# bing164/PL-VI-ORBSLAM3

Hardware: AMD Instinct MI355X
Metric: frames/sec ORB+LSD extract+match, 640×480 mono, 1/2/4/8 MI355X (higher is better)
Workload: dtype u8; 1 GPU; C1+C2+C3: ORB extract (1000 feats, 1.2, 8 levels, FAST 20/7) || LSD+LBD (200 lines, scale 0.8, 2 octaves) as one HIP-stream schedule, then ORB kNN-2 + LineMatcher::match vs previous frame; batch=3072, width=640, height=480, parallelism=sequence-sharded x1, gather=False, inflight=2

## Files before the change

include/plvi_frontend.h:

```cpp
#ifndef PLVI_FRONTEND_H
#define PLVI_FRONTEND_H

#include <stddef.h>
#include <stdint.h>

#ifdef __cplusplus
extern "C" {
#endif

enum {
  PLVI_OK = 0,
  PLVI_E_EMPTY = -1,
  PLVI_E_BADARG = -2,
  PLVI_E_CAPACITY = -3,
  PLVI_E_HIP = -4,
  PLVI_E_OVERFLOW = -5,
  PLVI_E_SIZE = -6,
  PLVI_E_CAPTURE = -7,
};

enum {
  PLVI_COMPAT_GAUSS_ROUNDED = 1,
  PLVI_COMPAT_RESIZE_V_GENERIC = 2,
  PLVI_COMPAT_EXP_CV_TABLE = 4,
// ... 52 lines not shown
                     int* cap);

int plvi_orb_pyramid_level(plvi_orb_extractor* h, int frame, int level, uint8_t* dst, int* w, int* hgt);

int plvi_orb_pyramid_device(plvi_orb_extractor* h, int level, const uint8_t** d_frame0, size_t* frame_stride, int* w,
                            int* hgt, int* nlevels);

int plvi_orb_scale_tables(plvi_orb_extractor* h, float* scale, float* inv_scale, float* sigma2, float* inv_sigma2);

int plvi_orb_level_quota(plvi_orb_extractor* h, int* quota);

int plvi_orb_profile(plvi_orb_extractor* h, int enable);
int plvi_orb_profile_read(plvi_orb_extractor* h, float* stage_ms, int* runs);

int plvi_orb_kernel_timing(plvi_orb_extractor* h, int enable);
int plvi_orb_kernel_timing_read(plvi_orb_extractor* h, float* total_ms, int* launches);
int plvi_orb_kernel_timing_read_kind(plvi_orb_extractor* h, int kind, float* total_ms, int* launches);
int plvi_orb_debug_node_cap(plvi_orb_extractor* h, int cap);

typedef struct plvi_line_extractor plvi_line_extractor;

typedef struct plvi_line_params {
  int nfeatures;
  int refine;
  float lsd_scale;
  int nlevels;
  float scale;
  int extractor;
  unsigned compat;
} plvi_line_params;

int plvi_lines_create(const plvi_line_params* p, int width, int height, int max_batch, int device,
                      plvi_line_extractor** out);
int plvi_lines_destroy(plvi_line_extractor* h);

int plvi_lines_extract(plvi_line_extractor* h, const uint8_t* img, int width, int height, size_t stride,
                       plvi_keyline* keylines, uint8_t* desc, double* line_fns, int cap, int* n);

int plvi_lines_extract_batch(plvi_line_extractor* h, const uint8_t* d_frames, int n_frames, size_t frame_stride,
                             size_t row_stride, void* stream);
int plvi_lines_outputs(plvi_line_extractor* h, plvi_keyline** d_kl, uint8_t** d_desc, double** d_fn, int** d_count,
                       int* cap);
int plvi_lines_errors(plvi_line_extractor* h, int* frame_flags, int* any, void* stream);

int plvi_lines_pyramid_level(plvi_line_extractor* h, int frame, int level, uint8_t* dst, int* w, int* hgt);

int plvi_lines_scale_tables(plvi_line_extractor* h, float* scale, float* inv_scale, float* sigma2, float* inv_sigma2);

int plvi_lines_profile(plvi_line_extractor* h, int enable);
int plvi_lines_debug_stats(plvi_line_extractor* h, unsigned long long* d_stats);
int plvi_lines_debug_mw_stats(plvi_line_extractor* h, int* d_stats);
int plvi_lines_debug_planes(plvi_line_extractor* h, int frame, int octave, float* deg, double* modgrad, float* cs,
                            int* sw, int* sh);
int plvi_lines_debug_sobel(plvi_line_extractor* h, int frame, int octave, short* dxdy, int* w, int* hgt);
int plvi_lines_debug_raw_lines(plvi_line_extractor* h, int frame, int octave, float* out, int cap, int* n);
int plvi_lines_profile_read(plvi_line_extractor* h, float* stage_ms, int* runs);
int plvi_lines_kernel_timing(plvi_line_extractor* h, int enable);
int plvi_lines_kernel_timing_read(plvi_line_extractor* h, float* total_ms, int* launches);
int plvi_lines_kernel_timing_read_kind(plvi_line_extractor* h, int kind, float* total_ms, int* launches);


int plvi_hamming_knn2_batch(const uint8_t* d_q, const int* d_nq, int nq_cap, const uint8_t* d_t, const int* d_nt,
                            int nt_cap, int n_pairs, int* d_idx0, int* d_d0, int* d_idx1, int* d_d1, void* stream);

int plvi_hamming_knn2(const uint8_t* q, int nq, const uint8_t* t, int nt, int* idx0, int* d0, int* idx1, int* d1);

int plvi_line_match_nnr(const uint8_t* desc1, int n1, const uint8_t* desc2, int n2, float nnr, int* matches_12);

int plvi_line_match(const uint8_t* desc1, int n1, const uint8_t* desc2, int n2, float nnr, int* matches_12);

int plvi_line_match_nnr_inout(const uint8_t* desc1, int n1, const uint8_t* desc2, int n2, float nnr, int* matches_12,
                              int n_prev);
int plvi_line_match_inout(const uint8_t* desc1, int n1, const uint8_t* desc2, int n2, float nnr, int* matches_12,
                          int n_prev);

int plvi_line_match_batch(const uint8_t* d_desc1, const int* d_n1, int cap1, const uint8_t* d_desc2, const int* d_n2,
                          int cap2, int n_pairs, float nnr, int* d_scratch, int* d_matches_12, int* d_nmatch,
                          void* stream);

int plvi_descriptor_distance_batch(const uint8_t* d_a, const uint8_t* d_b, int n, int line_matcher_quirk, int* d_out,
                                   void* stream);

int plvi_search_by_bow(float nnratio, int check_orientation, const uint8_t* kf_desc, const float* kf_angle,
                       const uint8_t* kf_live, int kf_n, const int* kf_node, const int* kf_off, int kf_nnodes,
                       const int* kf_idx, const uint8_t* f_desc, const float* f_angle, int f_n, const int* f_node,
                       const int* f_off, int f_nnodes, const int* f_idx, int* match_kf);

int plvi_search_by_bow_batch(int n_pairs, float nnratio, int check_orientation, int kf_cap, int f_cap, int node_cap,
                             const uint8_t* d_kf_desc, const float* d_kf_angle, const uint8_t* d_kf_live,
                             const int* d_kf_node, const int* d_kf_off, const int* d_kf_nnodes, const int* d_kf_idx,
                             const uint8_t* d_f_desc, const float* d_f_angle, const int* d_f_n, const int* d_f_node,
                             const int* d_f_off, const int* d_f_nnodes, const int* d_f_idx, int* d_match_kf,
                             int* d_nmatches, void* stream);

int plvi_search_by_bow_stereo(float nnratio, int check_orientation, const uint8_t* kf_desc, const float* kf_angle,
                              const uint8_t* kf_live, int kf_n, const int* kf_node, const int* kf_off, int kf_nnodes,
                              const int* kf_idx, const uint8_t* f_desc, const float* f_angle, int f_n,
                              const int* f_node, const int* f_off, int f_nnodes, const int* f_idx, int f_nleft,
                              int* match_kf);
int plvi_search_by_bow_stereo_batch(int n_pairs, float nnratio, int check_orientation, int kf_cap, int f_cap,
                                    int node_cap, const uint8_t* d_kf_desc, const float* d_kf_angle,
                                    const uint8_t* d_kf_live, const int* d_kf_node, const int* d_kf_off,
                                    const int* d_kf_nnodes, const int* d_kf_idx, const uint8_t* d_f_desc,
                                    const float* d_f_angle, const int* d_f_n, const int* d_f_node, const int* d_f_off,
                                    const int* d_f_nnodes, const int* d_f_idx, const int* d_f_nleft, int* d_match_kf,
                                    int* d_nmatches, void* stream);
// ... 547 lines not shown
```

pl-vi-orbslam3_amd/csrc/lines_device.h:

```cpp
#pragma once
#include <cstdint>

namespace plvi {

constexpr int kLineMaxOct = 2;
constexpr int kLsdRawCap = 8192;
constexpr int kPrepBands = 8;
constexpr int kPrepBandMax = 256;


struct LineOctDev {
    int w, h;
    long long off;
    long long plane;
    int sw, sh;
    long long soff;
    long long splane;
    int min_reg_size;
    float octaveScale;
    int maxWH;
    long long tabXofs, tabXa, tabYrow, tabYb;
    int xmax;
    long long tabStrips;
    int nstrips;
    long long tabBands1, tabBandsK;
    int lw, lh;
    long long loff, lplane;
};

struct LsdLine {
    float x1, y1, x2, y2;
};

struct LsdRegion {
    int start, n;
    double angle;
};

struct LsdPix {
    float deg;
    float c, s;
    float pad;
};

}
```

pl-vi-orbslam3_amd/csrc/lines_kernels.hpp:

```cpp
#include <hip/hip_runtime.h>

#include "lines_device.h"
#include "plvi_common.h"
#include "plvi_math.h"
#include "std_sort.h"

namespace plvi {

constexpr double kNotdef = -1024.0;
constexpr float kNotdefF = -1024.0f;
constexpr double kD2R = 3.14159265358979323846 / 180;
constexpr double kPi = 3.14159265358979323846;
constexpr double kLog10Of11 = 0x1.0a98b6050c56fp+0;

__global__ __launch_bounds__(256) void lsd_half_kernel(const uint8_t* __restrict__ src, size_t s_frame, size_t s_row,
                                                       uint8_t* __restrict__ dst, int dw, int dh, size_t d_frame) {
    const int f = blockIdx.y;
    const int i = blockIdx.x * 256 + threadIdx.x;
    if (i >= dw * dh) return;
    const int y = i / dw, x = i % dw;
    const uint8_t* S0 = src + (size_t)f * s_frame + (size_t)(2 * y) * s_row;
    const uint8_t* S1 = S0 + s_row;
    const int s = S0[2 * x] + S0[2 * x + 1] + S1[2 * x] + S1[2 * x + 1];
    const int simd = (dw / 8) * 8;
    int v = x < simd ? (s + 2) >> 2 : (int)__builtin_rintf((float)s * 0.25f);
    dst[(size_t)f * d_frame + (size_t)y * dw + x] = (uint8_t)min(max(v, 0), 255);
}

__device__ __forceinline__ int readlane_i(int v, int l) { return __builtin_amdgcn_readlane(v, l); }
__device__ __forceinline__ float readlane_f(float v, int l) {
    return __int_as_float(__builtin_amdgcn_readlane(__float_as_int(v), l));
}
__device__ __forceinline__ double readlane_d(double v, int l) {
    const long long b = __double_as_longlong(v);
    const int lo = __builtin_amdgcn_readlane((int)(b & 0xffffffff), l);
    const int hi = __builtin_amdgcn_readlane((int)(b >> 32), l);
    return __longlong_as_double(((long long)hi << 32) | (unsigned)lo);
}
__device__ __forceinline__ double shfl_d(double v, int src) {
    const long long b = __double_as_longlong(v);
    const int lo = __shfl((int)(b & 0xffffffff), src);
    const int hi = __shfl((int)(b >> 32), src);
    return __longlong_as_double(((long long)hi << 32) | (unsigned)lo);
}

__device__ __forceinline__ int dpp_from_right(int v) {
    return __builtin_amdgcn_update_dpp(0, v, 0x130, 0xf, 0xf, false);
}
__device__ __forceinline__ int dpp_from_left(int v) {
    return __builtin_amdgcn_update_dpp(0, v, 0x138, 0xf, 0xf, false);
}
__device__ __forceinline__ double dpp_from_right_d(double v) {
    const long long b = __double_as_longlong(v);
    const int lo = dpp_from_right((int)(b & 0xffffffff)), hi = dpp_from_right((int)(b >> 32));
    return __longlong_as_double(((long long)hi << 32) | (unsigned)lo);
}

__global__ __launch_bounds__(64) void lsd_prep_kernel(const uint8_t* __restrict__ src, size_t s_frame, size_t s_row,
                                                       int gw, int gh, int sw, int sh, const int4* __restrict__ strips,
                                                       const int4* __restrict__ bands,
                                                       const int* __restrict__ xofs, const float* __restrict__ xa,
                                                       int xmax, const int* __restrict__ yrow,
                                                       const float* __restrict__ yb, double k0, double k1, double k2,
                                                       double k3, double rho, float* __restrict__ pix,
                                                       double* __restrict__ modgrad, float2* __restrict__ pixcs,
                                                       size_t p_frame) {
    __shared__ int hostdx[64];
    const int4 sd = strips[blockIdx.x];
    const int f = blockIdx.y;
    const int4 bd = bands[blockIdx.z];
    const int dyA = bd.x, dyB = bd.y, ybase0 = bd.z;
    const int dyEnd = dyB < sh ? dyB + 1 : sh;
    const int X0 = sd.x, X1 = sd.y, gx0 = sd.z, nc = sd.w;
    const int lane = threadIdx.x;
    const int Lt = xofs[X0 + min(lane, nc - 1)] - gx0 + 3;
    hostdx[lane] = -1;
    __builtin_amdgcn_wave_barrier();
    __builtin_amdgcn_fence(__ATOMIC_ACQ_REL, "wavefront");
    if (lane < nc) hostdx[Lt] = X0 + lane;
    __builtin_amdgcn_wave_barrier();
    __builtin_amdgcn_fence(__ATOMIC_ACQ_REL, "wavefront");
    const int hdx = hostdx[lane];
    const bool interp = hdx >= 0 && hdx < xmax;
    const double a0 = interp ? (double)xa[2 * hdx] : 1.0, a1 = interp ? (double)xa[2 * hdx + 1] : 0.0;
    const uint8_t* S = src + (size_t)f * s_frame + reflect101(gx0 - 3 + lane, gw);
    const int nout = X1 - X0;
    float* P = pix + (size_t)f * p_frame + X0;
    double* M = modgrad + (size_t)f * p_frame + X0;
    float2* CS = pixcs + (size_t)f * p_frame + X0;
    const int yend = gh + 3;
    uint32_t pb[7];
#pragma unroll
    for (int k = 0; k < 7; ++k) pb[k] = S[(size_t)reflect101(ybase0 + k, gh) * s_row];
    double Hw[7];
    double Gprev = 0.0, Gprevn = 0.0, Sp = 0.0, Spn = 0.0;
    int dy = dyA;
    auto emit = [&](int y, double Sc, double Scn) {
        if (lane >= nout) return;
        const int x = X0 + lane;
        float deg = kNotdefF;
        double norm = 0.0;
        if (x < sw - 1 && y < sh - 1) {
            const double DA = Scn - Sp;
            const double BC = Spn - Sc;
            const double gx = DA + BC, gy = DA - BC;
            norm = __builtin_sqrt(rfma(gx, gx, gy * gy) / 4);
            if (!(norm <= rho)) deg = plvi_fast_atan2((float)gx, (float)-gy);
        }
        const size_t o = (size_t)y * sw + lane;
        P[o] = deg;
        M[o] = norm;
        if (deg != kNotdefF) {
            float ps, pc;
            plvi_sincosf_pos((float)((double)deg * kD2R), &ps, &pc);
            CS[o] = make_float2(pc, ps);
        }
    };
    for (int ybase = ybase0; ybase < yend && dy < dyEnd; ybase += 7) {
#pragma unroll
        for (int k = 0; k < 7; ++k) {
            const int y = ybase + k;
            if (y >= yend || dy >= dyEnd) break;
            const int v0 = (int)pb[k];
            if (y + 7 < yend) pb[k] = S[(size_t)reflect101(y + 7, gh) * s_row];
            const int r1 = dpp_from_right(v0), r2 = dpp_from_right(r1), r3 = dpp_from_right(r2);
            const int l1 = dpp_from_left(v0), l2 = dpp_from_left(l1), l3 = dpp_from_left(l2);
            double s = k0 * (double)l3;
            s += k1 * (double)l2;
            s += k2 * (double)l1;
            s += k3 * (double)v0;
            s += k2 * (double)r1;
            s += k1 * (double)r2;
            s += k0 * (double)r3;
            Hw[k] = s;
            const int g = y - 3;
            if (g < ybase0 + 3) continue;
            double G = k3 * Hw[(k + 4) % 7] + 0.0;
            G += k2 * (Hw[(k + 5) % 7] + Hw[(k + 3) % 7]);
            G += k1 * (Hw[(k + 6) % 7] + Hw[(k + 2) % 7]);
            G += k0 * (Hw[k] + Hw[(k + 1) % 7]);
            const double Gn = dpp_from_right_d(G);
            while (dy < dyEnd && yrow[2 * dy + 1] == g) {
                const bool same = yrow[2 * dy] == g;
                const double G0 = same ? G : Gprev, G0n = same ? Gn : Gprevn;
                const double b0 = (double)yb[2 * dy], b1 = (double)yb[2 * dy + 1];
                double H0, H1;
                if (interp) {
                    H0 = G0 * a0 + G0n * a1;
                    H1 = G * a0 + Gn * a1;
                } else {
                    H0 = G0 * 1.0;
                    H1 = G * 1.0;
                }
                const double Sv = H0 * b0 + H1 * b1;
                const double Sc = shfl_d(Sv, Lt);
                const double Scn = dpp_from_right_d(Sc);
                if (dy > dyA) emit(dy - 1, Sc, Scn);
                Sp = Sc;
                Spn = Scn;
                ++dy;
            }
            Gprev = G;
            Gprevn = Gn;
        }
    }
    if (dyB == sh) emit(sh - 1, 0.0, 0.0);
}


struct GrowCtx {
    const float* P;
    unsigned* gbits;
    lds_u32* bits;
    lds_u32* qlds;
    unsigned* qglob;
    lds_f32* win;
    int sw, sh, R, RB, wpr, wb, wbb, QL, ys;
};

typedef unsigned short plvi_u16x2 __attribute__((ext_vector_type(2)));
__device__ __forceinline__ unsigned long long dup_lanes(unsigned pv, int nb, int bp, int nx, int ny) {
    const unsigned pn1 = (unsigned)(nx + 1) | ((unsigned)(ny + 1) << 16);
    const int s = 3 * ny + nx + 4;
    unsigned long long dup = 0;
    for (int p2 = 0; p2 < nb - 1; ++p2) {
        const unsigned q2 = (unsigned)__builtin_amdgcn_readlane((int)pv, 9 * p2);
        const int t2 = 3 * (int)(q2 >> 16) + (int)(q2 & 0xffffu);
        const plvi_u16x2 d = __builtin_bit_cast(plvi_u16x2, pn1) - __builtin_bit_cast(plvi_u16x2, q2);
        const plvi_u16x2 m = __builtin_elementwise_max(d, (plvi_u16x2){2, 2});
        const bool hit = (p2 < bp) & (__builtin_bit_cast(unsigned, m) == 0x00020002u);
        const unsigned long long hm = 0ull - (unsigned long long)hit;
        dup |= (1ull << ((9 * p2 - t2 + s) & 63)) & hm;
    }
    return dup;
}

__device__ __forceinline__ unsigned long long ballot(bool b) { return __builtin_amdgcn_ballot_w64(b); }
__device__ __forceinline__ int mbcnt64(unsigned long long m) {
    return (int)__builtin_amdgcn_mbcnt_hi((unsigned)(m >> 32), __builtin_amdgcn_mbcnt_lo((unsigned)m, 0u));
}
__device__ __forceinline__ unsigned gload_l2(unsigned* p) {
    return __hip_atomic_load(p, __ATOMIC_RELAXED, __HIP_MEMORY_SCOPE_AGENT);
}
__device__ __forceinline__ void gstore_l2(unsigned* p, unsigned v) {
    __hip_atomic_store(p, v, __ATOMIC_RELAXED, __HIP_MEMORY_SCOPE_AGENT);
}
__device__ __forceinline__ void vm_drain() { __builtin_amdgcn_s_waitcnt(0); }

__device__ __forceinline__ bool used_get(const GrowCtx& g, int x, int y) {
    const bool inwin = y < g.wbb + g.RB;
    const int yy = inwin ? y : g.wbb;
    unsigned v = g.bits[(yy & (g.RB - 1)) * g.wpr + (x >> 5)];
    if (__builtin_expect(!inwin, 0)) v = gload_l2(g.gbits + (size_t)y * g.wpr + (x >> 5));
    return y < g.ys || ((v >> (x & 31)) & 1u);
}
__device__ __forceinline__ void used_set(const GrowCtx& g, int x, int y) {
    const unsigned b = 1u << (x & 31);
    if (__builtin_expect(y < g.wbb + g.RB, 1))
// ... 1133 lines not shown
```

pl-vi-orbslam3_amd/csrc/lines_pipeline.hip:

```cpp
#include <hip/hip_runtime.h>

#include <algorithm>
#include <cmath>
#include <cstdlib>
#include <cstring>
#include <memory>
#include <vector>

#include "lines_device.h"
#include "lines_kernels.hpp"
#include "lsd_grow_mw.hpp"
#include "plvi_common.h"

extern "C" int plvi_orb_internal_blur_event(plvi_orb_extractor* h, hipEvent_t ev);
extern "C" int plvi_orb_internal_stage_event(plvi_orb_extractor* h, int stage, hipEvent_t ev);

namespace plvi {

static inline int lround_h(float v) { return (int)lrintf(v); }
static inline int lround_h(double v) { return (int)lrint(v); }
static inline int lfloor_h(float v) { int i = (int)v; return i - (i > v); }

static double cv_exp64f(double x) {
    const double a0s = .9670371139572337719125840413672004409288e-2;
    const double k5 = .99999999999999999998285227504999 / a0s, k4 = .69314718055994546743029643825322 / a0s,
                 k3 = .24022650695886477918181338054308 / a0s, k2 = .55504108793649567998466049042729e-1 / a0s,
                 k1 = .96180973140732918010002372686186e-2 / a0s, k0 = .13369713757180123244806654839424e-2 / a0s;
    const double pre = 1.4426950408889634073599246810019 * 64;
    double y = x * pre;
    const int v = (int)lrint(y);
    int e = (v >> 6) + 1023;
    e = e < 0 ? 0 : e > 2047 ? 2047 : e;
    const double p2 = std::ldexp(1.0, e - 1023);
    const double tab = (double)exp2l((long double)(v & 63) / 64.0L) * a0s;
    y = (y - v) * (1. / 64);
    return p2 * tab * (((((k0 * y + k1) * y + k2) * y + k3) * y + k4) * y + k5);
}

static void gauss_kernel_f64(int n, double sigma, double* k, bool cvExp) {
    const double scale2X = -0.125 / (sigma * sigma);
    const int n2 = (n - 1) / 2;
    std::vector<double> values(n2 + 1);
    double sum = 0;
    for (int i = 0, x = 1 - n; i < n2; ++i, x += 2) {
        const double a = (double)(x * x) * scale2X;
        double t = cvExp ? cv_exp64f(a) : std::exp(a);
        values[i] = t;
        sum += t;
    }
    sum *= 2;
    sum += 1.0;
    const double mul1 = 1.0 / sum;
    for (int i = 0; i < n2; ++i) k[i] = k[n - 1 - i] = values[i] * mul1;
    k[n2] = 1.0 * mul1;
}

struct LinePipeline {
    plvi_line_params prm{};
    int W = 0, H = 0, Bcap = 0, device = 0, nOct = 0, fcap = 0;
    hipStream_t stream = nullptr;
    hipStream_t aux[2] = {nullptr, nullptr};
    hipEvent_t evSobelGo = nullptr;
    hipEvent_t evFork = nullptr, evPrep = nullptr, evSobel = nullptr, evOrb = nullptr, evCrit = nullptr,
               evBlur = nullptr, evGate = nullptr, evGrow2 = nullptr, evPair = nullptr;
    bool growAfterBlur = true, sobelWithGrow = false, growSplit = false;
    int sobelGate = -1;
    bool sobelAfterGrow = false;
    hipStream_t critStream = nullptr;
    hipStream_t crit2 = nullptr;
    hipStream_t octStream = nullptr;
    int orbAfterPrep = 1;
    std::vector<LineOctDev> oct;
    std::vector<float> scaleF, invScaleF;
    double SCALE = 0.8, prec = 0, rho = 0, min_length = 0;
    double gk[7]{};
    int lbdTaps[3] = {14, 62, 104};
    DevBuf d_oct, d_tabs, octImg, pix, modg, seedcs, gbits, qspill, regs, regpts, rawLines, nlines, klTmp, klOut, fnOut, cntOut, descOut, lbdBlur,
        lbdG, err, staging, mwOwn, mwSlot, mwGrow, sortPos;
    size_t qspillFrame = 0, gbitsFrame = 0, lbdPlaneTotal = 0;
    int lastFrames = 0;
    static constexpr int kStages = 5, kRing = 512;
    bool prof = false;
    int profRuns = 0;
    std::vector<hipEvent_t> evs;

    static constexpr int kKRing = 4096;
    bool ktime = false;
    int kn = 0;
    std::vector<hipEvent_t> kev;
    std::vector<hipEvent_t> kevS[3];
    int knS[3] = {0, 0, 0};
    int ktiming(int on) {
        if (on && kev.empty()) {
            kev.resize(2 * kKRing);
            for (auto& e : kev) PLVI_CHECK(hipEventCreate(&e));
            for (auto& v : kevS) {
                v.resize(2 * kKRing);
                for (auto& e : v) PLVI_CHECK(hipEventCreate(&e));
            }
        }
        ktime = on != 0;
        if (on) kn = knS[0] = knS[1] = knS[2] = 0;
        return PLVI_OK;
    }
    void ktimeS(int k, int edge, hipStream_t st) {
        if (!ktime || knS[k] >= kKRing) return;
        (void)hipEventRecord(kevS[k][2 * knS[k] + edge], st);
// ... 81 lines not shown
        SCALE = (double)p->lsd_scale;
        if (!(SCALE > 0) || SCALE > 1) return PLVI_E_BADARG;
        const double ANG_TH = 22.5, QUANT = 2.0, SIGMA_SCALE = 0.6;
        prec = M_PI * ANG_TH / 180;
        const double pp = ANG_TH / 180;
        rho = QUANT / std::sin(prec);
        min_length = 0.025 * std::min(W, H);
        const double sigma = (SCALE < 1) ? (SIGMA_SCALE / SCALE) : SIGMA_SCALE;
        const unsigned hk = (unsigned)std::ceil(sigma * std::sqrt(2 * 3.0 * std::log(10.0)));
        if (SCALE != 1 && 1 + 2 * hk != 7) return PLVI_E_BADARG;
        gauss_kernel_f64(7, sigma, gk, (p->compat & PLVI_COMPAT_EXP_CV_TABLE) != 0);
        if (SCALE == 1) gk[0] = gk[1] = gk[2] = 0.0, gk[3] = 1.0;
        lbdTaps[0] = 14;
        lbdTaps[1] = (p->compat & PLVI_COMPAT_GAUSS_ROUNDED) ? 63 : 62;
        lbdTaps[2] = (p->compat & PLVI_COMPAT_GAUSS_ROUNDED) ? 103 : 104;
        scaleF.assign(nOct, 1.f); invScaleF.assign(nOct, 1.f);
        for (int l = 0; l < nOct; ++l) {
            if (l > 0) scaleF[l] = scaleF[l - 1] * p->scale;
            invScaleF[l] = 1.0f / scaleF[l];
        }
        oct.resize(nOct);
        size_t imgOff = 0, sOff = 0, lOff = 0, maxSplane = 0;
        std::vector<uint8_t> tabs;
        auto put = [&](const void* src, size_t n) {
            size_t o = (tabs.size() + 15) & ~size_t(15);
            tabs.resize(o + n);
            std::memcpy(tabs.data() + o, src, n);
            return (long long)o;
        };
        for (int l = 0; l < nOct; ++l) {
            LineOctDev& d = oct[l];
            std::memset(&d, 0, sizeof(d));
            d.w = lround_h((float)W * invScaleF[l]);
            d.h = lround_h((float)H * invScaleF[l]);
            if (l > 0) {
                if (d.w * 2 != oct[l - 1].w || d.h * 2 != oct[l - 1].h) return PLVI_E_BADARG;
                if (std::fabs(scaleF[l] / scaleF[l - 1] - 2.0f) > 0) return PLVI_E_BADARG;
            }
            d.plane = (long long)d.w * d.h;
            d.off = (long long)imgOff;
            if (l > 0) imgOff += (size_t)d.plane * Bcap;
            d.sw = SCALE != 1 ? lround_h(d.w * SCALE) : d.w;
            d.sh = SCALE != 1 ? lround_h(d.h * SCALE) : d.h;
            d.splane = (long long)d.sw * d.sh;
            d.soff = (long long)sOff;
            sOff += (size_t)d.splane * Bcap;
            maxSplane = std::max(maxSplane, (size_t)d.splane);
            const double LOG_NT = rfma(5 * (std::log10((double)d.sw) + std::log10((double)d.sh)), 0.5,
                                       kLog10Of11);
            d.min_reg_size = (int)(-LOG_NT / std::log10(pp));
            d.octaveScale = (float)std::pow(p->scale, l);
            d.maxWH = std::max(d.w, d.h);
            {
                const double sx = 1. / SCALE, sy = 1. / SCALE;
                std::vector<int> xofs(d.sw), yrow(2 * d.sh);
                std::vector<float> xa(2 * d.sw), yb(2 * d.sh);
                int xmax = d.sw;
                for (int dx = 0; dx < d.sw; ++dx) {
                    float fx = (float)((dx + 0.5) * sx - 0.5);
                    int s = lfloor_h(fx);
                    fx -= s;
                    if (s < 0) { fx = 0; s = 0; }
                    if (s + 1 >= d.w) {
                        xmax = std::min(xmax, dx);
                        if (s >= d.w - 1) { fx = 0; s = d.w - 1; }
                    }
                    xofs[dx] = s;
                    xa[2 * dx] = 1.f - fx;
                    xa[2 * dx + 1] = fx;
                }
                for (int dy = 0; dy < d.sh; ++dy) {
                    float fy = (float)((dy + 0.5) * sy - 0.5);
                    int s = lfloor_h(fy);
                    fy -= s;
                    yrow[2 * dy] = std::min(std::max(s, 0), d.h - 1);
                    yrow[2 * dy + 1] = std::min(std::max(s + 1, 0), d.h - 1);
                    yb[2 * dy] = 1.f - fy;
                    yb[2 * dy + 1] = fy;
                }
                d.xmax = xmax;
                std::vector<int> strips;
                for (int X0 = 0; X0 < d.sw;) {
                    const int gx0 = xofs[X0];
                    int E = X0;
                    while (E < d.sw && xofs[E] + (E < xmax ? 1 : 0) - gx0 + 3 <= 60) ++E;
                    const int X1 = E == d.sw ? E : E - 1;
                    if (X1 <= X0) return PLVI_E_BADARG;
                    strips.insert(strips.end(), {X0, X1, gx0, E - X0});
                    X0 = X1;
                }
                for (int dy = 0; dy < d.sh; ++dy) {
                    const int r1 = yrow[2 * dy + 1], r0 = yrow[2 * dy];
                    if (r0 > r1 || r1 - r0 > 1 || (dy > 0 && r1 < yrow[2 * dy - 1])) return PLVI_E_BADARG;
                }
                d.nstrips = (int)strips.size() / 4;
                d.tabStrips = put(strips.data(), strips.size() * 4);
                for (int nb : {1, kPrepBands}) {
                    std::vector<int> bands;
                    for (int b = 0; b < nb; ++b) {
                        const int dyA = (int)((long long)d.sh * b / nb), dyB = (int)((long long)d.sh * (b + 1) / nb);
                        bands.insert(bands.end(), {dyA, dyB, dyA == 0 ? -3 : yrow[2 * dyA] - 3, 0});
                    }
                    (nb == 1 ? d.tabBands1 : d.tabBandsK) = put(bands.data(), bands.size() * 4);
                }
                d.tabXofs = put(xofs.data(), xofs.size() * 4);
                d.tabXa = put(xa.data(), xa.size() * 4);
                d.tabYrow = put(yrow.data(), yrow.size() * 4);
                d.tabYb = put(yb.data(), yb.size() * 4);
            }
            d.lw = l == 0 ? W : oct[l - 1].lw / 2;
            d.lh = l == 0 ? H : oct[l - 1].lh / 2;
            d.lplane = (long long)d.lw * d.lh;
            d.loff = (long long)lOff;
            lOff += (size_t)d.lplane * Bcap;
        }
        lbdPlaneTotal = lOff;
        qspillFrame = (maxSplane + 1) & ~size_t(1);
        for (auto& d : oct) gbitsFrame = std::max(gbitsFrame, (size_t)d.sh * (size_t)((d.sw + 31) / 32));
        if (d_oct.alloc(sizeof(LineOctDev) * nOct) || d_tabs.alloc(tabs.size())) return PLVI_E_HIP;
        PLVI_CHECK(hipMemcpy(d_oct.p, oct.data(), sizeof(LineOctDev) * nOct, hipMemcpyHostToDevice));
        PLVI_CHECK(hipMemcpy(d_tabs.p, tabs.data(), tabs.size(), hipMemcpyHostToDevice));
        {
            float gL[21], gG[63];
            double u = (7 * 3 - 1) / 2, sg = (7 * 2 + 1) / 2, inv = -1 / (2 * sg * sg);
            for (int i = 0; i < 21; ++i) { double dis = i - u; gL[i] = (float)std::exp(dis * dis * inv); }
            u = (9 * 7 - 1) / 2; sg = u; inv = -1 / (2 * sg * sg);
            for (int i = 0; i < 63; ++i) { double dis = i - u; gG[i] = (float)std::exp(dis * dis * inv); }
            static const unsigned char comb[64] = {0, 1, 0, 2, 0, 3, 0, 4, 0, 5, 0, 6, 1, 2, 1, 3, 1, 4, 1, 5, 1, 6,
                                                   2, 3, 2, 4, 2, 5, 2, 6, 2, 7, 2, 8, 3, 4, 3, 5, 3, 6, 3, 7, 3, 8,
                                                   4, 5, 4, 6, 4, 7, 4, 8, 5, 6, 5, 7, 5, 8, 6, 7, 6, 8, 7, 8};
            PLVI_CHECK(hipMemcpyToSymbol(HIP_SYMBOL(c_gaussL), gL, sizeof(gL)));
            PLVI_CHECK(hipMemcpyToSymbol(HIP_SYMBOL(c_gaussG), gG, sizeof(gG)));
            PLVI_CHECK(hipMemcpyToSymbol(HIP_SYMBOL(c_comb), comb, sizeof(comb)));
        }
        if (octImg.alloc(std::max<size_t>(imgOff, 16)) || pix.alloc(sizeof(float) * sOff) ||
            modg.alloc(sizeof(double) * sOff) || seedcs.alloc(sizeof(float2) * sOff) ||
            gbits.alloc(sizeof(unsigned) * gbitsFrame * nOct * Bcap) || qspill.alloc(sizeof(unsigned) * qspillFrame * nOct * Bcap) ||
            rawLines.alloc(sizeof(LsdLine) * (size_t)kLsdRawCap * nOct * Bcap) ||
            regs.alloc(sizeof(LsdRegion) * (size_t)kLsdRawCap * nOct * Bcap) ||
            regpts.alloc(sizeof(unsigned) * qspillFrame * nOct * Bcap) ||
            nlines.alloc(sizeof(int) * nOct * Bcap) || klTmp.alloc(sizeof(plvi_keyline) * (size_t)kKlCap * Bcap) ||
            sortPos.alloc(sizeof(unsigned short) * 2 * (size_t)kKlCap * Bcap) ||
            klOut.alloc(sizeof(plvi_keyline) * (size_t)fcap * Bcap) || fnOut.alloc(sizeof(double) * 3 * fcap * Bcap) ||
            cntOut.alloc(sizeof(int) * Bcap) || descOut.alloc((size_t)32 * fcap * Bcap) ||
            lbdBlur.alloc((size_t)W * H * Bcap) || lbdG.alloc(sizeof(short2) * lbdPlaneTotal) ||
            err.alloc(sizeof(int) * Bcap) || staging.alloc((size_t)W * H))
            return PLVI_E_HIP;
        PLVI_CHECK(hipMemset(err.p, 0, sizeof(int) * Bcap));
        size_t maxSw = 0;
        for (auto& d : oct) maxSw = std::max(maxSw, (size_t)d.sw);
        const size_t wprMax = (maxSw + 31) / 32;
        size_t budget = 6 * 1024;
        if (const char* e = getenv("PLVI_GROW_LDS")) budget = (size_t)atol(e);
        budget = std::min<size_t>(budget, 160 * 1024);
        growRB = 64;
        if (const char* e = getenv("PLVI_GROW_RB")) growRB = atoi(e);
        if (growRB < 2 || (growRB & (growRB - 1)) || growRB > 1024) return PLVI_E_BADARG;
        growQL = budget >= 32 * 1024 ? 1024 : 256;
        const size_t fixed = (size_t)growQL * sizeof(unsigned) + (size_t)growRB * wprMax * sizeof(unsigned);
        const size_t perRow = maxSw * sizeof(float);
        growR = 0;
// ... 54 lines not shown
    unsigned long long* growStats = nullptr;

    int profile(int on) {
        if (on && evs.empty()) {
            evs.resize((size_t)kRing * (kStages + 1));
            for (auto& e : evs) PLVI_CHECK(hipEventCreate(&e));
        }
        prof = on != 0;
        profRuns = 0;
        return PLVI_OK;
    }
    void mark(int s, hipStream_t st) {
        if (prof && profRuns < kRing) (void)hipEventRecord(evs[(size_t)profRuns * (kStages + 1) + s], st);
    }
    int profile_read(float* ms, int* runs) {
        for (int k = 0; k < kStages; ++k) ms[k] = 0.f;
        for (int r = 0; r < profRuns; ++r) {
            PLVI_CHECK(hipEventSynchronize(evs[(size_t)r * (kStages + 1) + kStages]));
            for (int k = 0; k < kStages; ++k) {
                float t = 0.f;
                PLVI_CHECK(hipEventElapsedTime(&t, evs[(size_t)r * (kStages + 1) + k],
                                               evs[(size_t)r * (kStages + 1) + k + 1]));
                ms[k] += t;
            }
        }
        if (runs) *runs = profRuns;
        return PLVI_OK;
    }

    void launch_prep(const uint8_t* d_frames, int nf, size_t frame_stride, size_t row_stride, hipStream_t st,
                     int lFirst = 0, int lEnd = -1) {
        const uint8_t* T = d_tabs.as<uint8_t>();
        if (lEnd < 0) lEnd = nOct;
        for (int l = 1; l < nOct && lFirst == 0; ++l) {
            const LineOctDev& d = oct[l];
            const uint8_t* s = l == 1 ? d_frames : octImg.as<uint8_t>() + oct[l - 1].off;
            const size_t sf = l == 1 ? frame_stride : (size_t)oct[l - 1].plane;
            const size_t sr = l == 1 ? row_stride : (size_t)oct[l - 1].w;
            hipLaunchKernelGGL(lsd_half_kernel, dim3((d.w * d.h + 255) / 256, nf), dim3(256), 0, st, s, sf, sr,
                               octImg.as<uint8_t>() + d.off, d.w, d.h, (size_t)d.plane);
        }
        if (lFirst == 0) mark(1, st);
        for (int l = lFirst; l < lEnd; ++l) {
            const LineOctDev& d = oct[l];
            const uint8_t* s = l == 0 ? d_frames : octImg.as<uint8_t>() + d.off;
            const size_t sf = l == 0 ? frame_stride : (size_t)d.plane;
            const size_t sr = l == 0 ? row_stride : (size_t)d.w;
            const bool kt = ktime && kn < kKRing;
            if (kt) (void)hipEventRecord(kev[2 * kn], st);
            const bool banded = nf <= kPrepBandMax;
            hipLaunchKernelGGL(lsd_prep_kernel, dim3(d.nstrips, nf, banded ? kPrepBands : 1), dim3(64), 0, st, s, sf,
                               sr, d.w, d.h, d.sw, d.sh, (const int4*)(T + d.tabStrips),
                               (const int4*)(T + (banded ? d.tabBandsK : d.tabBands1)), (const int*)(T + d.tabXofs),
                               (const float*)(T + d.tabXa), d.xmax, (const int*)(T + d.tabYrow),
                               (const float*)(T + d.tabYb), gk[0], gk[1], gk[2], gk[3], rho,
                               pix.as<float>() + d.soff, modg.as<double>() + d.soff, seedcs.as<float2>() + d.soff,
                               (size_t)d.splane);
            if (kt) {
                (void)hipEventRecord(kev[2 * kn + 1], st);
                ++kn;
            }
        }
        if (lEnd == nOct) mark(2, st);
    }

    void launch_grow(int nf, int oBase, int oCount, hipStream_t st) {
        if (nf <= mwMaxFrames) {
            auto mwK = mwStats ? lsd_grow_mw_kernel<kMwWaves, true> : lsd_grow_mw_kernel<kMwWaves, false>;
            hipLaunchKernelGGL(mwK, dim3(oCount * nf), dim3(kMwWaves * 64), mwSmem, st, d_oct.as<LineOctDev>(),
                               (const float*)pix.as<float>(), (const float2*)seedcs.as<float2>(),
                               mwOwn.as<unsigned>(), mwOwnTask, mwGrow.as<unsigned>(), mwSlot.as<unsigned>(),
                               qspill.as<unsigned>(), qspillFrame, prec, regs.as<LsdRegion>(), regpts.as<unsigned>(),
                               qspillFrame, nlines.as<int>(), err.as<int>(), mwSlots, nOct, oBase, oCount, mwStats, nf,
                               mwStats && PLVI_MW_DIAG ? mwEpoch.as<int>() : nullptr);
            return;
        }
        const bool fixedWin = growR == 0 && growRB == kGrowRB && growQL == kGrowQL;
        const int tpwWant = growTPW > 0 ? growTPW : (inSchedule && nf >= 2048 ? 2 : 1);
        const int tpw = tpwWant > 1 && !growStats && fixedWin ? tpwWant : 1;
        auto growK = growStats ? (fixedWin ? lsd_grow_kernel<true, true> : lsd_grow_kernel<true, false>)
                               : (fixedWin ? (tpw > 1 ? lsd_grow_kernel<false, true, true> : lsd_grow_kernel<false, true>)
                                           : lsd_grow_kernel<false, false>);
        const int waves = (oCount * nf + tpw - 1) / tpw;
        hipLaunchKernelGGL(growK, dim3((waves + growWPW - 1) / growWPW), dim3(64 * growWPW),
                           growSmem * growWPW, st, d_oct.as<LineOctDev>(),
                           (const float*)pix.as<float>(), (const double*)modg.as<double>(),
                           (const float2*)seedcs.as<float2>(), gbits.as<unsigned>(), gbitsFrame,
                           qspill.as<unsigned>(), qspillFrame, prec, regs.as<LsdRegion>(), regpts.as<unsigned>(),
                           qspillFrame, nlines.as<int>(), err.as<int>(), growR, growRB, growQL, nOct, oBase, oCount,
                           growStats, nf, (int)growSmem, growWPW);
    }
    void launch_rect(int nf, int oBase, int oCount, hipStream_t st) {
        const int bx = nf <= 16 ? 8 : nf < kRectLargeNf ? kRectLaneBlocks : kRectLaneBlocksLarge;
        auto rectK = nf <= kRectSmallNf ? lsd_rect_lanes_kernel<kRectUSmall> : lsd_rect_lanes_kernel<kRectU>;
        ktimeS(2, 0, st);
        hipLaunchKernelGGL(rectK, dim3(bx, nf, oCount), dim3(256), 0, st, d_oct.as<LineOctDev>(),
                           (const double*)modg.as<double>(), (const LsdRegion*)regs.as<LsdRegion>(),
                           (const unsigned*)regpts.as<unsigned>(), qspillFrame, (const int*)nlines.as<int>(), prec,
                           SCALE, rawLines.as<LsdLine>(), oBase, nOct, qspill.as<double>(), qspillFrame / 2,
                           (int)(qspillFrame / 2));
        ktimeS(2, 1, st);
    }
    void launch_grow_assemble(int nf, hipStream_t st, bool grown = false, bool rect0 = false) {
        if (!grown) launch_grow(nf, 0, nOct, st);
        launch_rect(nf, 0, rect0 ? 1 : nOct, st);
        mark(3, st);
        hipLaunchKernelGGL(line_assemble_kernel, dim3(nf), dim3(256), 0, st, d_oct.as<LineOctDev>(), nOct,
// ... 358 lines not shown
        const float s = P.scaleF[i];
        const float s2 = i > 0 ? s * s : 1.0f;
        if (scale) scale[i] = s;
        if (inv_scale) inv_scale[i] = P.invScaleF[i];
        if (sigma2) sigma2[i] = s2;
        if (inv_sigma2) inv_sigma2[i] = 1.0f / s2;
    }
    return PLVI_OK;
}

extern "C" int plvi_lines_profile(plvi_line_extractor* h, int enable) {
    if (!h) return PLVI_E_BADARG;
    PLVI_CHECK(hipSetDevice(h->p().device));
    return h->p().profile(enable);
}

extern "C" int plvi_lines_profile_read(plvi_line_extractor* h, float* stage_ms, int* runs) {
    if (!h || !stage_ms) return PLVI_E_BADARG;
    PLVI_CHECK(hipSetDevice(h->p().device));
    return h->p().profile_read(stage_ms, runs);
}

extern "C" int plvi_lines_debug_stats(plvi_line_extractor* h, unsigned long long* d_stats) {
    if (!h) return PLVI_E_BADARG;
    h->p().growStats = d_stats;
    return PLVI_OK;
}

extern "C" int plvi_lines_debug_mw_stats(plvi_line_extractor* h, int* d_stats) {
    if (!h) return PLVI_E_BADARG;
    h->p().mwStats = d_stats;
    if (PLVI_MW_DIAG && d_stats && !h->p().mwEpoch.p &&
        h->p().mwEpoch.alloc(sizeof(int) * 32 * h->p().gbitsFrame * (size_t)h->p().mwMaxFrames * h->p().nOct))
        return PLVI_E_HIP;
    return PLVI_OK;
}

extern "C" int plvi_lines_debug_planes(plvi_line_extractor* h, int frame, int octave, float* deg, double* modgrad,
                                       float* cs, int* sw, int* sh) {
    if (!h || octave < 0 || octave >= h->p().nOct || frame < 0 || frame >= h->p().Bcap) return PLVI_E_BADARG;
    LinePipeline& P = h->p();
    PLVI_CHECK(hipSetDevice(P.device));
    const plvi::LineOctDev& d = P.oct[octave];
    const size_t n = (size_t)d.splane, o = (size_t)d.soff + (size_t)frame * n;
    if (sw) *sw = d.sw;
    if (sh) *sh = d.sh;
    PLVI_CHECK(hipDeviceSynchronize());
    if (deg) PLVI_CHECK(hipMemcpy(deg, P.pix.as<float>() + o, n * sizeof(float), hipMemcpyDeviceToHost));
    if (modgrad) PLVI_CHECK(hipMemcpy(modgrad, P.modg.as<double>() + o, n * sizeof(double), hipMemcpyDeviceToHost));
    if (cs) PLVI_CHECK(hipMemcpy(cs, P.seedcs.as<float2>() + o, n * sizeof(float2), hipMemcpyDeviceToHost));
    return PLVI_OK;
}

extern "C" int plvi_lines_debug_raw_lines(plvi_line_extractor* h, int frame, int octave, float* out, int cap, int* n) {
    if (!h || octave < 0 || octave >= h->p().nOct || frame < 0 || frame >= h->p().Bcap || cap < 0) return PLVI_E_BADARG;
    LinePipeline& P = h->p();
    PLVI_CHECK(hipSetDevice(P.device));
    PLVI_CHECK(hipDeviceSynchronize());
    const size_t task = (size_t)frame * P.nOct + octave;
    int cnt = 0;
    PLVI_CHECK(hipMemcpy(&cnt, P.nlines.as<int>() + task, sizeof(int), hipMemcpyDeviceToHost));
    cnt = std::min(cnt, plvi::kLsdRawCap);
    if (n) *n = cnt;
    if (cnt > cap) return PLVI_E_CAPACITY;
    if (out && cnt > 0)
        PLVI_CHECK(hipMemcpy(out, P.rawLines.as<plvi::LsdLine>() + task * plvi::kLsdRawCap,
                             sizeof(plvi::LsdLine) * cnt, hipMemcpyDeviceToHost));
    return PLVI_OK;
}

extern "C" int plvi_lines_debug_sobel(plvi_line_extractor* h, int frame, int octave, short* dxdy, int* w, int* hgt) {
    if (!h || octave < 0 || octave >= h->p().nOct || frame < 0 || frame >= h->p().Bcap) return PLVI_E_BADARG;
    LinePipeline& P = h->p();
    PLVI_CHECK(hipSetDevice(P.device));
    const plvi::LineOctDev& d = P.oct[octave];
    if (w) *w = d.lw;
    if (hgt) *hgt = d.lh;
    PLVI_CHECK(hipDeviceSynchronize());
    if (dxdy)
        PLVI_CHECK(hipMemcpy(dxdy, P.lbdG.as<short2>() + d.loff + (size_t)frame * d.lplane,
                             (size_t)d.lplane * sizeof(short2), hipMemcpyDeviceToHost));
    return PLVI_OK;
}

extern "C" int plvi_lines_kernel_timing(plvi_line_extractor* h, int enable) {
    if (!h) return PLVI_E_BADARG;
    PLVI_CHECK(hipSetDevice(h->p().device));
    return h->p().ktiming(enable);
}

extern "C" int plvi_lines_kernel_timing_read(plvi_line_extractor* h, float* total_ms, int* launches) {
    if (!h) return PLVI_E_BADARG;
    PLVI_CHECK(hipSetDevice(h->p().device));
    return h->p().ktiming_read(total_ms, launches);
}

extern "C" int plvi_lines_kernel_timing_read_kind(plvi_line_extractor* h, int kind, float* total_ms, int* launches) {
    if (!h) return PLVI_E_BADARG;
    PLVI_CHECK(hipSetDevice(h->p().device));
    return h->p().ktiming_read_kind(kind, total_ms, launches);
}
```

Baseline: 61630 frames/s.

## Precompute LSD prep row schedule table and remove per-row branching in prep kernel

Result: no change. 61520 frames/s (-0.2%).

```diff
diff --git a/include/plvi_frontend.h b/include/plvi_frontend.h
--- a/include/plvi_frontend.h
+++ b/include/plvi_frontend.h
@@ -128,6 +128,8 @@
 int plvi_lines_debug_mw_stats(plvi_line_extractor* h, int* d_stats);
 int plvi_lines_debug_planes(plvi_line_extractor* h, int frame, int octave, float* deg, double* modgrad, float* cs,
                             int* sw, int* sh);
+int plvi_lines_prep_row_table(int h, float lsd_scale, int* sh, int* yrow, float* yb, int* rows, int rows_cap,
+                              int* nrows);
 int plvi_lines_debug_sobel(plvi_line_extractor* h, int frame, int octave, short* dxdy, int* w, int* hgt);
 int plvi_lines_debug_raw_lines(plvi_line_extractor* h, int frame, int octave, float* out, int cap, int* n);
 int plvi_lines_profile_read(plvi_line_extractor* h, float* stage_ms, int* runs);
diff --git a/pl-vi-orbslam3_amd/csrc/lines_device.h b/pl-vi-orbslam3_amd/csrc/lines_device.h
--- a/pl-vi-orbslam3_amd/csrc/lines_device.h
+++ b/pl-vi-orbslam3_amd/csrc/lines_device.h
@@ -7,6 +7,7 @@
 constexpr int kLsdRawCap = 8192;
 constexpr int kPrepBands = 8;
 constexpr int kPrepBandMax = 256;
+constexpr int kPrepRowPad = 24;
 
 
 struct LineOctDev {
@@ -24,6 +25,7 @@
     long long tabStrips;
     int nstrips;
     long long tabBands1, tabBandsK;
+    long long tabPrepRows;
     int lw, lh;
     long long loff, lplane;
 };
diff --git a/pl-vi-orbslam3_amd/csrc/lines_kernels.hpp b/pl-vi-orbslam3_amd/csrc/lines_kernels.hpp
--- a/pl-vi-orbslam3_amd/csrc/lines_kernels.hpp
+++ b/pl-vi-orbslam3_amd/csrc/lines_kernels.hpp
@@ -1,4 +1,6 @@
 #include <hip/hip_runtime.h>
+
+#include <type_traits>
 
 #include "lines_device.h"
 #include "plvi_common.h"
@@ -50,9 +52,15 @@
 __device__ __forceinline__ int dpp_from_left(int v) {
     return __builtin_amdgcn_update_dpp(0, v, 0x138, 0xf, 0xf, false);
 }
-__device__ __forceinline__ double dpp_from_right_d(double v) {
+__device__ __forceinline__ int dpp_bc_from_right(int v) {
+    return __builtin_amdgcn_mov_dpp(v, 0x130, 0xf, 0xf, true);
+}
+__device__ __forceinline__ int dpp_bc_from_left(int v) {
+    return __builtin_amdgcn_mov_dpp(v, 0x138, 0xf, 0xf, true);
+}
+__device__ __forceinline__ double dpp_bc_from_right_d(double v) {
     const long long b = __double_as_longlong(v);
-    const int lo = dpp_from_right((int)(b & 0xffffffff)), hi = dpp_from_right((int)(b >> 32));
+    const int lo = dpp_bc_from_right((int)(b & 0xffffffff)), hi = dpp_bc_from_right((int)(b >> 32));
     return __longlong_as_double(((long long)hi << 32) | (unsigned)lo);
 }
 
@@ -60,7 +68,8 @@
                                                        int gw, int gh, int sw, int sh, const int4* __restrict__ strips,
                                                        const int4* __restrict__ bands,
                                                        const int* __restrict__ xofs, const float* __restrict__ xa,
-                                                       int xmax, const int* __restrict__ yrow,
+                                                       int xmax, const int4* __restrict__ rows,
+                                                       const int* __restrict__ yrow,
                                                        const float* __restrict__ yb, double k0, double k1, double k2,
                                                        double k3, double rho, float* __restrict__ pix,
                                                        double* __restrict__ modgrad, float2* __restrict__ pixcs,
@@ -69,7 +78,7 @@
     const int4 sd = strips[blockIdx.x];
     const int f = blockIdx.y;
     const int4 bd = bands[blockIdx.z];
-    const int dyA = bd.x, dyB = bd.y, ybase0 = bd.z;
+    const int dyA = bd.x, dyB = bd.y, ybase0 = bd.z, ngroups = bd.w;
     const int dyEnd = dyB < sh ? dyB + 1 : sh;
     const int X0 = sd.x, X1 = sd.y, gx0 = sd.z, nc = sd.w;
     const int lane = threadIdx.x;
@@ -83,18 +92,21 @@
     const int hdx = hostdx[lane];
     const bool interp = hdx >= 0 && hdx < xmax;
     const double a0 = interp ? (double)xa[2 * hdx] : 1.0, a1 = interp ? (double)xa[2 * hdx + 1] : 0.0;
-    const uint8_t* S = src + (size_t)f * s_frame + reflect101(gx0 - 3 + lane, gw);
+    const uint8_t* S = src + (size_t)f * s_frame;
+    const int col = reflect101(gx0 - 3 + lane, gw);
     const int nout = X1 - X0;
     float* P = pix + (size_t)f * p_frame + X0;
     double* M = modgrad + (size_t)f * p_frame + X0;
     float2* CS = pixcs + (size_t)f * p_frame + X0;
-    const int yend = gh + 3;
+    const int4* R = rows + (ybase0 + 3);
+    const int* Y = (const int*)(rows + (gh + kPrepRowPad)) + (ybase0 + 3);
     uint32_t pb[7];
 #pragma unroll
-    for (int k = 0; k < 7; ++k) pb[k] = S[(size_t)reflect101(ybase0 + k, gh) * s_row];
+    for (int k = 0; k < 7; ++k) pb[k] = S[(size_t)Y[k] * s_row + col];
     double Hw[7];
-    double Gprev = 0.0, Gprevn = 0.0, Sp = 0.0, Spn = 0.0;
-    int dy = dyA;
+#pragma unroll
+    for (int k = 0; k < 7; ++k) Hw[k] = 0.0;
+    double Hprev = 0.0, Sp = 0.0, Spn = 0.0;
     auto emit = [&](int y, double Sc, double Scn) {
         if (lane >= nout) return;
         const int x = X0 + lane;
@@ -116,15 +128,27 @@
             CS[o] = make_float2(pc, ps);
         }
     };
-    for (int ybase = ybase0; ybase < yend && dy < dyEnd; ybase += 7) {
+    auto complete = [&](int d, bool same, double b0, double b1, double Hc) {
+        const double H0 = same ? Hc : Hprev;
+        const double Sv = H0 * b0 + Hc * b1;
+        const double Sc = shfl_d(Sv, Lt);
+        const double Scn = dpp_bc_from_right_d(Sc);
+        if (d > dyA) emit(d - 1, Sc, Scn);
+        Sp = Sc;
+        Spn = Scn;
+    };
+    int4 rc = make_int4(0, 0, 0, 0);
+    auto group = [&](const int4* Rg, const int* Yg, auto first) {
+        constexpr bool kFirst = decltype(first)::value;
+        uint32_t pn[7];
+#pragma unroll
+        for (int k = 0; k < 7; ++k) pn[k] = S[(size_t)Yg[7 + k] * s_row + col];
+        if (kFirst) rc = Rg[7 + 6];
 #pragma unroll
         for (int k = 0; k < 7; ++k) {
-            const int y = ybase + k;
-            if (y >= yend || dy >= dyEnd) break;
             const int v0 = (int)pb[k];
-            if (y + 7 < yend) pb[k] = S[(size_t)reflect101(y + 7, gh) * s_row];
-            const int r1 = dpp_from_right(v0), r2 = dpp_from_right(r1), r3 = dpp_from_right(r2);
-            const int l1 = dpp_from_left(v0), l2 = dpp_from_left(l1), l3 = dpp_from_left(l2);
+            const int r1 = dpp_bc_from_right(v0), r2 = dpp_bc_from_right(r1), r3 = dpp_bc_from_right(r2);
+            const int l1 = dpp_bc_from_left(v0), l2 = dpp_bc_from_left(l1), l3 = dpp_bc_from_left(l2);
             double s = k0 * (double)l3;
             s += k1 * (double)l2;
             s += k2 * (double)l1;
@@ -133,37 +157,35 @@
             s += k1 * (double)r2;
             s += k0 * (double)r3;
             Hw[k] = s;
-            const int g = y - 3;
-            if (g < ybase0 + 3) continue;
-            double G = k3 * Hw[(k + 4) % 7] + 0.0;
-            G += k2 * (Hw[(k + 5) % 7] + Hw[(k + 3) % 7]);
-            G += k1 * (Hw[(k + 6) % 7] + Hw[(k + 2) % 7]);
-            G += k0 * (Hw[k] + Hw[(k + 1) % 7]);
-            const double Gn = dpp_from_right_d(G);
-            while (dy < dyEnd && yrow[2 * dy + 1] == g) {
-                const bool same = yrow[2 * dy] == g;
-                const double G0 = same ? G : Gprev, G0n = same ? Gn : Gprevn;
-                const double b0 = (double)yb[2 * dy], b1 = (double)yb[2 * dy + 1];
-                double H0, H1;
-                if (interp) {
-                    H0 = G0 * a0 + G0n * a1;
-                    H1 = G * a0 + Gn * a1;
-                } else {
-                    H0 = G0 * 1.0;
-                    H1 = G * 1.0;
+            if (!kFirst || k == 6) {
+                double G = k3 * Hw[(k + 4) % 7] + 0.0;
+                G += k2 * (Hw[(k + 5) % 7] + Hw[(k + 3) % 7]);
+                G += k1 * (Hw[(k + 6) % 7] + Hw[(k + 2) % 7]);
+                G += k0 * (Hw[k] + Hw[(k + 1) % 7]);
+                const double Gn = dpp_bc_from_right_d(G);
+                double Hc;
+                if (interp)
+                    Hc = G * a0 + Gn * a1;
+                else
+                    Hc = G * 1.0;
+                const int fl = rc.x, n = fl & 0xff, d = fl >> 12;
+                const float fb0 = __int_as_float(rc.y), fb1 = __int_as_float(rc.z);
+                if (n != 0) {
+                    if (d >= dyA && d < dyEnd)
+                        complete(d, (fl & 0x100) != 0, (double)fb0, (double)fb1, Hc);
+                    if (n > 1 && d + 1 >= dyA && d + 1 < dyEnd)
+                        complete(d + 1, yrow[2 * d + 2] == yrow[2 * d + 3], (double)yb[2 * d + 2], (double)yb[2 * d + 3],
+                                 Hc);
                 }
-                const double Sv = H0 * b0 + H1 * b1;
-                const double Sc = shfl_d(Sv, Lt);
-                const double Scn = dpp_from_right_d(Sc);
-                if (dy > dyA) emit(dy - 1, Sc, Scn);
-                Sp = Sc;
-                Spn = Scn;
-                ++dy;
-            }
-            Gprev = G;
-            Gprevn = Gn;
-        }
-    }
+                rc = Rg[7 + k + 1];
+                Hprev = Hc;
+            }
+        }
+#pragma unroll
+        for (int k = 0; k < 7; ++k) pb[k] = pn[k];
+    };
+    group(R, Y, std::true_type{});
+    for (int gi = 1; gi < ngroups; ++gi) group(R + 7 * gi, Y + 7 * gi, std::false_type{});
     if (dyB == sh) emit(sh - 1, 0.0, 0.0);
 }
 
diff --git a/pl-vi-orbslam3_amd/csrc/lines_pipeline.hip b/pl-vi-orbslam3_amd/csrc/lines_pipeline.hip
--- a/pl-vi-orbslam3_amd/csrc/lines_pipeline.hip
+++ b/pl-vi-orbslam3_amd/csrc/lines_pipeline.hip
@@ -53,6 +53,50 @@
     const double mul1 = 1.0 / sum;
     for (int i = 0; i < n2; ++i) k[i] = k[n - 1 - i] = values[i] * mul1;
     k[n2] = 1.0 * mul1;
+}
+
+static void lsd_resize_rows(int h, int sh, double SCALE, std::vector<int>& yrow, std::vector<float>& yb) {
+    const double sy = 1. / SCALE;
+    yrow.resize(2 * (size_t)sh);
+    yb.resize(2 * (size_t)sh);
+    for (int dy = 0; dy < sh; ++dy) {
+        float fy = (float)((dy + 0.5) * sy - 0.5);
+        int s = lfloor_h(fy);
+        fy -= s;
+        yrow[2 * dy] = std::min(std::max(s, 0), h - 1);
+        yrow[2 * dy + 1] = std::min(std::max(s + 1, 0), h - 1);
+        yb[2 * dy] = 1.f - fy;
+        yb[2 * dy + 1] = fy;
+    }
+}
+
+static bool lsd_prep_row_table(int h, int sh, const std::vector<int>& yrow, const std::vector<float>& yb,
+                               std::vector<int>& rows) {
+    if (sh >= (1 << 19)) return false;
+    for (int dy = 0; dy < sh; ++dy) {
+        const int r1 = yrow[2 * dy + 1], r0 = yrow[2 * dy];
+        if (r0 > r1 || r1 - r0 > 1 || (dy > 0 && r1 < yrow[2 * dy - 1])) return false;
+    }
+    const int N = h + kPrepRowPad;
+    rows.assign(5 * (size_t)N, 0);
+    int dy = 0;
+    for (int t = 0; t < N; ++t) {
+        const int g = t - 13, p = t - 3;
+        int* e = &rows[4 * (size_t)t];
+        if (g >= 0 && g < h) {
+            while (dy < sh && yrow[2 * dy + 1] < g) ++dy;
+            int n = 0;
+            while (dy + n < sh && yrow[2 * (dy + n) + 1] == g) ++n;
+            if (n > 2) return false;
+            if (n > 0) {
+                e[0] = n | (yrow[2 * dy] == g ? 0x100 : 0) | (dy << 12);
+                std::memcpy(&e[1], &yb[2 * dy], sizeof(float));
+                std::memcpy(&e[2], &yb[2 * dy + 1], sizeof(float));
+            }
+        }
+        rows[4 * (size_t)N + t] = std::min(std::max(p <= h + 2 ? reflect101(p, h) : h - 1, 0), h - 1);
+    }
+    return true;
 }
 
 struct LinePipeline {
@@ -240,9 +284,9 @@
             d.octaveScale = (float)std::pow(p->scale, l);
             d.maxWH = std::max(d.w, d.h);
             {
-                const double sx = 1. / SCALE, sy = 1. / SCALE;
-                std::vector<int> xofs(d.sw), yrow(2 * d.sh);
-                std::vector<float> xa(2 * d.sw), yb(2 * d.sh);
+                const double sx = 1. / SCALE;
+                std::vector<int> xofs(d.sw), yrow, rows;
+                std::vector<float> xa(2 * d.sw), yb;
                 int xmax = d.sw;
                 for (int dx = 0; dx < d.sw; ++dx) {
                     float fx = (float)((dx + 0.5) * sx - 0.5);
@@ -257,15 +301,7 @@
                     xa[2 * dx] = 1.f - fx;
                     xa[2 * dx + 1] = fx;
                 }
-                for (int dy = 0; dy < d.sh; ++dy) {
-                    float fy = (float)((dy + 0.5) * sy - 0.5);
-                    int s = lfloor_h(fy);
-                    fy -= s;
-                    yrow[2 * dy] = std::min(std::max(s, 0), d.h - 1);
-                    yrow[2 * dy + 1] = std::min(std::max(s + 1, 0), d.h - 1);
-                    yb[2 * dy] = 1.f - fy;
-                    yb[2 * dy + 1] = fy;
-                }
+                lsd_resize_rows(d.h, d.sh, SCALE, yrow, yb);
                 d.xmax = xmax;
                 std::vector<int> strips;
                 for (int X0 = 0; X0 < d.sw;) {
@@ -277,17 +313,19 @@
                     strips.insert(strips.end(), {X0, X1, gx0, E - X0});
                     X0 = X1;
                 }
-                for (int dy = 0; dy < d.sh; ++dy) {
-                    const int r1 = yrow[2 * dy + 1], r0 = yrow[2 * dy];
-                    if (r0 > r1 || r1 - r0 > 1 || (dy > 0 && r1 < yrow[2 * dy - 1])) return PLVI_E_BADARG;
-                }
+                if (!lsd_prep_row_table(d.h, d.sh, yrow, yb, rows)) return PLVI_E_BADARG;
                 d.nstrips = (int)strips.size() / 4;
                 d.tabStrips = put(strips.data(), strips.size() * 4);
                 for (int nb : {1, kPrepBands}) {
                     std::vector<int> bands;
                     for (int b = 0; b < nb; ++b) {
                         const int dyA = (int)((long long)d.sh * b / nb), dyB = (int)((long long)d.sh * (b + 1) / nb);
-                        bands.insert(bands.end(), {dyA, dyB, dyA == 0 ? -3 : yrow[2 * dyA] - 3, 0});
+                        const int ybase0 = dyA == 0 ? -3 : yrow[2 * dyA] - 3;
+                        const int dyLast = std::max(dyA, (dyB < d.sh ? dyB + 1 : d.sh) - 1);
+                        const int nsteps = yrow[2 * dyLast + 1] + 3 + 1 - ybase0;
+                        const int ngroups = (nsteps + 6) / 7;
+                        if (ybase0 + 3 + 7 * ngroups + 7 >= d.h + kPrepRowPad) return PLVI_E_BADARG;
+                        bands.insert(bands.end(), {dyA, dyB, ybase0, ngroups});
                     }
                     (nb == 1 ? d.tabBands1 : d.tabBandsK) = put(bands.data(), bands.size() * 4);
                 }
@@ -295,6 +333,7 @@
                 d.tabXa = put(xa.data(), xa.size() * 4);
                 d.tabYrow = put(yrow.data(), yrow.size() * 4);
                 d.tabYb = put(yb.data(), yb.size() * 4);
+                d.tabPrepRows = put(rows.data(), rows.size() * 4);
             }
             d.lw = l == 0 ? W : oct[l - 1].lw / 2;
             d.lh = l == 0 ? H : oct[l - 1].lh / 2;
@@ -455,7 +494,8 @@
             hipLaunchKernelGGL(lsd_prep_kernel, dim3(d.nstrips, nf, banded ? kPrepBands : 1), dim3(64), 0, st, s, sf,
                                sr, d.w, d.h, d.sw, d.sh, (const int4*)(T + d.tabStrips),
                                (const int4*)(T + (banded ? d.tabBandsK : d.tabBands1)), (const int*)(T + d.tabXofs),
-                               (const float*)(T + d.tabXa), d.xmax, (const int*)(T + d.tabYrow),
+                               (const float*)(T + d.tabXa), d.xmax, (const int4*)(T + d.tabPrepRows),
+                               (const int*)(T + d.tabYrow),
                                (const float*)(T + d.tabYb), gk[0], gk[1], gk[2], gk[3], rho,
                                pix.as<float>() + d.soff, modg.as<double>() + d.soff, seedcs.as<float2>() + d.soff,
                                (size_t)d.splane);
@@ -920,6 +960,27 @@
     return PLVI_OK;
 }
 
+extern "C" int plvi_lines_prep_row_table(int h, float lsd_scale, int* sh, int* yrow, float* yb, int* rows,
+                                         int rows_cap, int* nrows) {
+    const double SCALE = (double)lsd_scale;
+    if (h < 1 || !(SCALE > 0) || SCALE > 1) return PLVI_E_BADARG;
+    const int s = SCALE != 1 ? plvi::lround_h(h * SCALE) : h;
+    if (s < 1) return PLVI_E_BADARG;
+    if (sh) *sh = s;
+    if (nrows) *nrows = h + plvi::kPrepRowPad;
+    std::vector<int> yr, rw;
+    std::vector<float> b;
+    plvi::lsd_resize_rows(h, s, SCALE, yr, b);
+    if (!plvi::lsd_prep_row_table(h, s, yr, b, rw)) return PLVI_E_BADARG;
+    if (yrow) std::memcpy(yrow, yr.data(), yr.size() * sizeof(int));
+    if (yb) std::memcpy(yb, b.data(), b.size() * sizeof(float));
+    if (rows) {
+        if (rows_cap < h + plvi::kPrepRowPad) return PLVI_E_CAPACITY;
+        std::memcpy(rows, rw.data(), rw.size() * sizeof(int));
+    }
+    return PLVI_OK;
+}
+
 extern "C" int plvi_lines_debug_raw_lines(plvi_line_extractor* h, int frame, int octave, float* out, int cap, int* n) {
     if (!h || octave < 0 || octave >= h->p().nOct || frame < 0 || frame >= h->p().Bcap || cap < 0) return PLVI_E_BADARG;
     LinePipeline& P = h->p();
```
